# gillesdegottex/percivaltts

Measured on AMD Instinct MI355X. Metric: acoustic frames/sec per WGAN-GP critic+gen step, higher is better.
Workload: dtype f32

## Files before the change

### percivaltts_amd/csrc/dense.hip

```cpp
#include "common.h"
#include <cstdlib>

namespace ptts {
namespace dns {

typedef __bf16 bf16x8 __attribute__((ext_vector_type(8)));
typedef __bf16 bf16x4 __attribute__((ext_vector_type(4)));
typedef __bf16 bf16x2 __attribute__((ext_vector_type(2)));
typedef float f32x4 __attribute__((ext_vector_type(4)));
typedef float f32x2 __attribute__((ext_vector_type(2)));
typedef unsigned u32x2 __attribute__((ext_vector_type(2)));
typedef unsigned short u16;

constexpr int THREADS = 512;
constexpr int NBLK = 256;
constexpr int BK = 32;

#define DNS_PRODUCTS(X) X(2, 0) X(1, 1) X(0, 2) X(1, 0) X(0, 1) X(0, 0)
#define DNS_PRODUCTS_NPL(NPL, X) do { if (NPL == 3) { X(2, 0) X(1, 1) X(0, 2) X(1, 0) X(0, 1) } X(0, 0) } while (0)

__device__ __forceinline__ unsigned pk_bf16(float a, float b) {
    return __builtin_bit_cast(unsigned, __builtin_convertvector((f32x2){a, b}, bf16x2));
}
__device__ __forceinline__ void split3_pair(float a, float b, unsigned& p1, unsigned& p2, unsigned& p3) {
    p1 = pk_bf16(a, b);
    const float ra = a - __builtin_bit_cast(float, p1 << 16), rb = b - __builtin_bit_cast(float, p1 & 0xffff0000u);
    p2 = pk_bf16(ra, rb);
    const float sa = ra - __builtin_bit_cast(float, p2 << 16), sb = rb - __builtin_bit_cast(float, p2 & 0xffff0000u);
    p3 = pk_bf16(sa, sb);
}
__device__ __forceinline__ float max_fast(float a, float b) {
    float r;
    asm("v_max_f32 %0, %1, %2" : "=v"(r) : "v"(a), "v"(b));
    return r;
}

__global__ __launch_bounds__(256) void split3_dense_weight_kernel(const float* __restrict__ w, long long ldw, int K, int N,
                                                                  int transposed, u16* __restrict__ planes, int NT, int KS) {
    const long long idx = (long long)blockIdx.x * 256 + threadIdx.x;
    if (idx >= (long long)NT * KS * 64) return;
    const int lane = (int)(idx & 63);
    const long long t = idx >> 6;
    const int ks = (int)(t % KS), nt = (int)(t / KS);
    const int n = nt * 16 + (lane & 15), k0 = ks * 32 + (lane >> 4) * 8;
    float v[8];
#pragma unroll
    for (int e = 0; e < 8; ++e) {
        const int k = k0 + e;
        v[e] = (n < N && k < K) ? (transposed ? w[(long long)n * ldw + k] : w[(long long)k * ldw + n]) : 0.f;
    }
    unsigned q[3][4];
#pragma unroll
    for (int h = 0; h < 4; ++h) split3_pair(v[2 * h], v[2 * h + 1], q[0][h], q[1][h], q[2][h]);
    const size_t ps = (size_t)NT * KS * 512;
// ... 123 lines not shown
constexpr int SPL_ROW = 256 + 2;
__global__ __launch_bounds__(256) void split3_dense_weight_strided_lds_kernel(SplitStridedArgs a) {
    __shared__ float tile[32 * SPL_ROW];
    const int z = blockIdx.y, ks = blockIdx.x % a.KS, cb = blockIdx.x / a.KS;
    const float* __restrict__ w = a.w + (long long)z * a.stride_w;
    u16* __restrict__ planes = a.planes + (long long)z * a.stride_p;
    const int lane = threadIdx.x & 63, wave = threadIdx.x >> 6;
    const int n0 = cb * 256;
#pragma unroll
    for (int j = 0; j < 8; ++j) {
        const int r = wave + 4 * j, k = ks * 32 + r, n = n0 + 4 * lane;
        f32x4 v = {0.f, 0.f, 0.f, 0.f};
        if (k < a.K && n < a.N) v = *reinterpret_cast<const f32x4*>(w + (long long)k * a.ldw + n);
        float* d = tile + r * SPL_ROW + 4 * lane;
        d[0] = v[0]; d[1] = v[1]; d[2] = v[2]; d[3] = v[3];
    }
    __syncthreads();
    const size_t ps = (size_t)a.NT * a.KS * 512;
    const int li = lane & 15, lg = lane >> 4;
#pragma unroll
    for (int j = 0; j < 4; ++j) {
        const int ntl = wave + 4 * j;
        const int nt = cb * 16 + ntl;
        if (nt >= a.NT) continue;
        float v[8];
#pragma unroll
        for (int e = 0; e < 8; ++e) v[e] = tile[(8 * lg + e) * SPL_ROW + 16 * ntl + li];
        unsigned q[3][4];
#pragma unroll
        for (int h = 0; h < 4; ++h) split3_pair(v[2 * h], v[2 * h + 1], q[0][h], q[1][h], q[2][h]);
        const size_t idx = ((size_t)nt * a.KS + ks) * 64 + lane;
#pragma unroll
        for (int p = 0; p < 3; ++p)
            *reinterpret_cast<uint4*>(planes + p * ps + idx * 8) = make_uint4(q[p][0], q[p][1], q[p][2], q[p][3]);
    }
}

#ifndef DNS_DEPTH
#define DNS_DEPTH 2
#endif
struct DenseArgs {
    const float* A; const float* mask_src; const float* in_scale; const float* in_shift;
    const u16* planes; const float* bias; const float* out_mask; float* C;
    int M, N, K, NT, KS;
    long long lda, ldc;
    float alpha, out_alpha;
    int accumulate, has_affine, vec_out;
    const float* res; int res_rows; long long ldr;
    long long bsA, bsP, bsC;
    double* stats;
    const float* om_scale; const float* om_shift;
};

template <int MODE, bool AFFINE, int MT, int NPL>
__global__ __launch_bounds__(THREADS) void dense_bf16x6_kernel(DenseArgs g) {
    if (gridDim.z > 1) {
        g.A += (long long)blockIdx.z * g.bsA;
        g.planes += (long long)blockIdx.z * g.bsP;
        g.C += (long long)blockIdx.z * g.bsC;
    }
    constexpr int TBM = 16 * MT;
    constexpr int NA = (TBM * 8 + THREADS - 1) / THREADS;
    constexpr int ROWS = NA * THREADS / 8;
    constexpr int PL = ROWS * BK;
    constexpr bool MASK = MODE == PTTS_IN_MASKMUL;
    __shared__ __attribute__((aligned(16))) u16 As[2][NPL * PL];
    const int tid = threadIdx.x, lane = tid & 63;
    const int wave = __builtin_amdgcn_readfirstlane(tid >> 6);
    const int li = lane & 15, lg = lane >> 4;
    const int m0 = blockIdx.x * TBM, n0 = blockIdx.y * NBLK;
    const int KS = g.KS;
    const bool wave_live = n0 + 32 * wave < g.N;

    const int kq = tid & 7;
    const float* pa[NA]; const float* pm[NA]; bool oka[NA]; int dst[NA];
#pragma unroll
    for (int j = 0; j < NA; ++j) {
        const int row = (tid + j * THREADS) >> 3;
        oka[j] = row < TBM && m0 + row < g.M;
        const long long base = (long long)(oka[j] ? m0 + row : 0) * g.lda + 4 * kq;
        pa[j] = g.A + base;
        pm[j] = MASK ? g.mask_src + base : nullptr;
        dst[j] = row * BK + ((((kq >> 1) ^ ((row >> 1) & 2))) << 3) + (kq & 1) * 4;
    }
    struct Stage { f32x4 va[NA], vm[MASK ? NA : 1], sc, sh; bool kok; };
    auto load_a = [&](int s, Stage& sg) {
        const int k = s * BK + 4 * kq;
        sg.kok = k < g.K;
        const int ko = sg.kok ? s * BK : -4 * kq;
#pragma unroll
        for (int j = 0; j < NA; ++j) {
            sg.va[j] = *reinterpret_cast<const f32x4*>(pa[j] + ko);
            if (MASK) sg.vm[j] = *reinterpret_cast<const f32x4*>(pm[j] + ko);
        }
        if (AFFINE) {
            sg.sc = *reinterpret_cast<const f32x4*>(g.in_scale + (sg.kok ? k : 0));
            sg.sh = *reinterpret_cast<const f32x4*>(g.in_shift + (sg.kok ? k : 0));
        }
    };
    auto commit = [&](const Stage& sg, u16* as) {
        const f32x4 z4 = {0.f, 0.f, 0.f, 0.f};
#pragma unroll
        for (int j = 0; j < NA; ++j) {
            f32x4 a = sg.va[j];
            if (MODE == PTTS_IN_LRELU) {
                if (AFFINE) a = a * sg.sc + sg.sh;
// ... 34 lines not shown

    f32x4 acc[MT][2];
#pragma unroll
    for (int i = 0; i < MT; ++i) { acc[i][0] = f32x4{0.f, 0.f, 0.f, 0.f}; acc[i][1] = f32x4{0.f, 0.f, 0.f, 0.f}; }
    const int boff = li * BK + ((lg ^ ((li >> 1) & 2)) << 3);
    auto mfma_rows = [&](const u16* as, const bf16x8 (&wf)[2][NPL], int i0, int i1) {
#pragma unroll
        for (int i = i0; i < i1; ++i) {
            bf16x8 bf[NPL];
#pragma unroll
            for (int p = 0; p < NPL; ++p) bf[p] = *reinterpret_cast<const bf16x8*>(as + p * PL + boff + i * 16 * BK);
#define DNS_MM(PA, PW)                                                                                    \
            acc[i][0] = __builtin_amdgcn_mfma_f32_16x16x32_bf16(wf[0][PW < NPL ? PW : 0], bf[PA < NPL ? PA : 0], acc[i][0], 0, 0, 0);    \
            acc[i][1] = __builtin_amdgcn_mfma_f32_16x16x32_bf16(wf[1][PW < NPL ? PW : 0], bf[PA < NPL ? PA : 0], acc[i][1], 0, 0, 0);
            DNS_PRODUCTS_NPL(NPL, DNS_MM);
#undef DNS_MM
        }
    };

    constexpr int DEPTH = DNS_DEPTH;
    Stage sg[DEPTH];
    bf16x8 wc[2][NPL], wn[2][NPL];
#pragma unroll
    for (int j = 0; j < DEPTH; ++j) load_a(j, sg[j]);
    load_w(0, wc);
    commit(sg[0], As[0]);
    load_a(DEPTH, sg[0]);
    __syncthreads();
    auto step = [&](int s, int cut, Stage& nx) {
        const u16* as = As[s & 1];
        load_w(s + 1 < KS ? s + 1 : s, wn);
        mfma_rows(as, wc, 0, cut);
        commit(nx, As[(s + 1) & 1]);
        load_a(s + 1 + DEPTH, nx);
        mfma_rows(as, wc, cut, MT);
#pragma unroll
        for (int j = 0; j < 2; ++j)
#pragma unroll
            for (int p = 0; p < NPL; ++p) wc[j][p] = wn[j][p];
        __syncthreads();
    };
    auto run = [&](int cut) {
        int s = 0;
        for (; s + DEPTH <= KS; s += DEPTH) {
#pragma unroll
            for (int j = 0; j < DEPTH; ++j) step(s + j, cut, sg[(j + 1) % DEPTH]);
        }
#pragma unroll
        for (int j = 0; j < DEPTH; ++j)
            if (s + j < KS) step(s + j, cut, sg[(j + 1) % DEPTH]);
    };
    if (wave < 4) run(2); else run(MT - 2);
    if (!wave_live) return;
    const bool interior = m0 + TBM <= g.M;
    if (!g.vec_out) {
#pragma unroll
        for (int j = 0; j < 2; ++j)
#pragma unroll
            for (int i = 0; i < MT; ++i) {
                const int m = m0 + 16 * i + li;
                if (m >= g.M) continue;
#pragma unroll
                for (int e = 0; e < 4; ++e) {
                    const int n = n0 + 32 * wave + 16 * j + 4 * lg + e;
                    if (n >= g.N) continue;
                    const long long off = (long long)m * g.ldc + n;
                    float v = acc[i][j][e] + (g.bias ? g.bias[n] : 0.f);
                    if (g.out_mask) v *= g.out_mask[off] > 0.f ? 1.f : g.out_alpha;
                    if (g.res) { int mr = m; while (mr >= g.res_rows) mr -= g.res_rows; v += g.res[(long long)mr * g.ldr + n]; }
                    g.C[off] = v;
                }
            }
        return;
    }
#pragma unroll
    for (int j = 0; j < 2; ++j) {
        const int n = n0 + 32 * wave + 16 * j + 4 * lg;
        if (n >= g.N) continue;
        f32x4 bv = {0.f, 0.f, 0.f, 0.f};
        if (g.bias) bv = *reinterpret_cast<const f32x4*>(g.bias + n);
        const long long off0 = (long long)(m0 + li) * g.ldc + n;
        auto res_at = [&](int m) { int mr = m; while (mr >= g.res_rows) mr -= g.res_rows; return g.res + (long long)mr * g.ldr + n; };
        f32x4 ssum = {0.f, 0.f, 0.f, 0.f}, ssq = {0.f, 0.f, 0.f, 0.f};
        f32x4 osc = {1.f, 1.f, 1.f, 1.f}, osh = {0.f, 0.f, 0.f, 0.f};
        if (g.om_scale) { osc = *reinterpret_cast<const f32x4*>(g.om_scale + n); osh = *reinterpret_cast<const f32x4*>(g.om_shift + n); }
        auto aff_store = [&](f32x4& v, const f32x4& z) {
#pragma unroll
            for (int e = 0; e < 4; ++e) {
                const float gd = v[e] * ((z[e] * osc[e] + osh[e]) > 0.f ? 1.f : g.out_alpha);
                ssum[e] += gd * z[e]; ssq[e] += gd;
                v[e] = gd * osc[e];
            }
        };
        if (interior) {
            f32x4 mk[MT], old[MT];
            if (g.out_mask) {
#pragma unroll
                for (int i = 0; i < MT; ++i) mk[i] = *reinterpret_cast<const f32x4*>(g.out_mask + off0 + (long long)16 * i * g.ldc);
            }
            if (g.res) {
#pragma unroll
                for (int i = 0; i < MT; ++i) old[i] = *reinterpret_cast<const f32x4*>(res_at(m0 + 16 * i + li));
            }
#pragma unroll
            for (int i = 0; i < MT; ++i) {
                f32x4 v = acc[i][j] + bv;
                if (g.om_scale) {
                    aff_store(v, mk[i]);
                } else if (g.out_mask) {
#pragma unroll
                    for (int e = 0; e < 4; ++e) v[e] = v[e] * (mk[i][e] > 0.f ? 1.f : g.out_alpha);
                }
                if (g.res) v += old[i];
                if (g.stats && !g.om_scale) { ssum += v; ssq += v * v; }
                *reinterpret_cast<f32x4*>(g.C + off0 + (long long)16 * i * g.ldc) = v;
            }
        } else {
#pragma unroll
            for (int i = 0; i < MT; ++i) {
                const int m = m0 + 16 * i + li;
                if (m >= g.M) continue;
                const long long off = off0 + (long long)16 * i * g.ldc;
                f32x4 v = acc[i][j] + bv;
                if (g.out_mask) {
                    const f32x4 mk = *reinterpret_cast<const f32x4*>(g.out_mask + off);
                    if (g.om_scale) {
                        aff_store(v, mk);
                    } else {
#pragma unroll
                        for (int e = 0; e < 4; ++e) v[e] = v[e] * (mk[e] > 0.f ? 1.f : g.out_alpha);
                    }
                }
                if (g.res) v += *reinterpret_cast<const f32x4*>(res_at(m));
                if (g.stats && !g.om_scale) { ssum += v; ssq += v * v; }
                *reinterpret_cast<f32x4*>(g.C + off) = v;
            }
        }
        if (g.stats) {
#pragma unroll
            for (int e = 0; e < 4; ++e)
#pragma unroll
                for (int m = 1; m < 16; m <<= 1) { ssum[e] += __shfl_xor(ssum[e], m, 64); ssq[e] += __shfl_xor(ssq[e], m, 64); }
            if (li == 0) {
                double* row = g.stats + (size_t)blockIdx.x * 2 * g.N;
#pragma unroll
                for (int e = 0; e < 4; ++e) { row[n + e] = (double)ssum[e]; row[g.N + n + e] = (double)ssq[e]; }
            }
        }
    }
}

static int pick_mt(int M, int col_blocks) {
    static int forced = -1;
    if (forced < 0) { const char* e = getenv("PTTS_DENSE_MT"); forced = e ? atoi(e) : 0; }
    if (forced >= 4 && forced <= 8) return forced;
    int best = 8; double best_eff = -1.0;
    for (int mt = 4; mt <= 8; ++mt) {
        const long long blocks = (long long)((M + 16 * mt - 1) / (16 * mt)) * col_blocks;
        const long long rounds = (blocks + 255) / 256;
        const double eff = (double)M * col_blocks / (double)(rounds * 256 * 16 * mt);
        if (eff > best_eff + 1e-9) { best_eff = eff; best = mt; }
    }
    return best;
}


typedef short s16x4 __attribute__((ext_vector_type(4)));
typedef s16x4 __attribute__((address_space(3)))* lds_s16x4_ptr;
__device__ __forceinline__ bf16x4 tr_read(const u16* p) {
    return __builtin_bit_cast(bf16x4, __builtin_amdgcn_ds_read_tr16_b64_v4i16((lds_s16x4_ptr)(p)));
}
__device__ __forceinline__ bf16x8 cat8(bf16x4 a, bf16x4 b) { return __builtin_shufflevector(a, b, 0, 1, 2, 3, 4, 5, 6, 7); }

struct WgradArgs {
    const float* A; const float* dY; const float* mask_src; const float* in_scale; const float* in_shift;
    float* partials;
    int Kin, N, M;
    long long lda, ldb;
    float alpha;
    int tiles_n, steps_total, split;
};

constexpr int WT = 128;
constexpr int WROW = WT;
constexpr int WPL = 32 * WROW;
constexpr int WPART = WT * WT + WT;

template <int MODE, bool AFFINE, int NPL>
__global__ __launch_bounds__(THREADS) void dense_wgrad_bf16x6_kernel(WgradArgs g) {
    constexpr bool MASK = MODE == PTTS_IN_MASKMUL;
    extern __shared__ __attribute__((aligned(16))) u16 lds_w[];
    const int tid = threadIdx.x, lane = tid & 63;
    const int wave = __builtin_amdgcn_readfirstlane(tid >> 6);
    const int li = lane & 15, lg = lane >> 4;
    const int tile = blockIdx.y, tk = tile / g.tiles_n, tn = tile - tk * g.tiles_n;
    const int k0 = tk * WT, n0 = tn * WT;
    const int per = (g.steps_total + g.split - 1) / g.split;
    const int s_begin = blockIdx.x * per, s_end = min(g.steps_total, s_begin + per);
    const int nsteps = max(0, s_end - s_begin);

    const int c4 = tid & 31;
    const bool a_ok = k0 + 4 * c4 < g.Kin, d_ok = n0 + 4 * c4 < g.N;
    const float* pa = g.A + (a_ok ? k0 + 4 * c4 : 0);
    const float* pm = MASK ? g.mask_src + (a_ok ? k0 + 4 * c4 : 0) : nullptr;
    const float* pd = g.dY + (d_ok ? n0 + 4 * c4 : 0);
    int dst[2];
#pragma unroll
    for (int j = 0; j < 2; ++j) {
        const int row = (tid + j * THREADS) >> 5;
        dst[j] = row * WROW + ((((c4 >> 2) + row + 4 * (row >> 3)) & 7) << 4) + (c4 & 3) * 4;
    }
    f32x4 sc = {1.f, 1.f, 1.f, 1.f}, sh = {0.f, 0.f, 0.f, 0.f};
    if (AFFINE && a_ok) { sc = *reinterpret_cast<const f32x4*>(g.in_scale + k0 + 4 * c4); sh = *reinterpret_cast<const f32x4*>(g.in_shift + k0 + 4 * c4); }
    struct Stage { f32x4 va[2], vm[MASK ? 2 : 1], vd[2]; bool ok[2]; };
// ... 285 lines not shown
}

extern "C" int ptts_dense_bf16x6_stats(const float* A, const void* planes, const float* bias, float* C, int M, int N, int K,
                                       long long lda, long long ldc, int in_mode, const float* in_scale, const float* in_shift,
                                       float alpha, double* stats, int capacity_rows, int* nrows_out, void* stream) {
    PTTS_REQUIRE(stats && nrows_out && capacity_rows > 0, "dense_bf16x6_stats: no room for the sums");
    return dense_launch(A, planes, bias, C, M, N, K, lda, ldc, in_mode, in_scale, in_shift, nullptr, alpha, nullptr, 0, 0, nullptr,
                        stats, capacity_rows, nrows_out, stream);
}
extern "C" int ptts_dense_bf16x6_bwd_affine(const float* A, const void* planes, float* C, int M, int N, int K, long long lda, long long ldc,
                                            const float* z, const float* scale, const float* shift, float alpha,
                                            double* stats, int capacity_rows, int* nrows_out, void* stream) {
    PTTS_REQUIRE(z && scale && shift && stats && nrows_out && capacity_rows > 0, "dense_bf16x6_bwd_affine: null pointer");
    PTTS_REQUIRE((((uintptr_t)scale | (uintptr_t)shift) & 15) == 0, "dense_bf16x6_bwd_affine: scale / shift must be 16-byte aligned");
    g_om_scale = scale; g_om_shift = shift;
    const int rc = dense_launch(A, planes, nullptr, C, M, N, K, lda, ldc, PTTS_IN_NONE, nullptr, nullptr, nullptr, alpha, nullptr, 0, 0, z,
                                stats, capacity_rows, nrows_out, stream);
    g_om_scale = g_om_shift = nullptr;
    return rc;
}
extern "C" int ptts_dense_bf16x6_stats_rows(int M, int N) {
    if (M <= 0 || N <= 0) return 0;
    const int mt = pick_mt(M, (N + NBLK - 1) / NBLK);
    return (M + 16 * mt - 1) / (16 * mt);
}

static int dense_launch(const float* A, const void* planes, const float* bias, float* C, int M, int N, int K,
                        long long lda, long long ldc, int in_mode, const float* in_scale, const float* in_shift,
                        const float* mask_src, float alpha, const float* res, int res_rows, long long ldr,
                        const float* out_mask, double* stats, int stats_capacity_rows, int* stats_rows_out, void* stream) {
    const int accumulate = res != nullptr;
    PTTS_REQUIRE(!res || (res_rows > 0 && ldr >= N && M <= 8LL * res_rows), "dense_bf16x6: bad residual (rows %d, ldr %lld)", res_rows, ldr);
    PTTS_REQUIRE(A && planes && C, "dense_bf16x6: null matrix");
    PTTS_REQUIRE(ptts_dense_bf16x6_supported(M, N, K, lda, ldc), "dense_bf16x6: unsupported shape M=%d N=%d K=%d lda=%lld ldc=%lld (K and lda must be multiples of 4)", M, N, K, lda, ldc);
    PTTS_REQUIRE(lda >= K && ldc >= N, "dense_bf16x6: bad leading dims");
    PTTS_REQUIRE(in_mode >= 0 && in_mode <= 2, "dense_bf16x6: bad in_mode %d", in_mode);
    PTTS_REQUIRE((in_scale == nullptr) == (in_shift == nullptr), "dense_bf16x6: scale/shift must come together");
    PTTS_REQUIRE(in_mode != PTTS_IN_MASKMUL || mask_src, "dense_bf16x6: MASKMUL needs mask_src");
    PTTS_REQUIRE(in_mode == PTTS_IN_LRELU || !in_scale, "dense_bf16x6: scale/shift need PTTS_IN_LRELU");
    PTTS_REQUIRE(!(out_mask && bias), "dense_bf16x6: out_mask with bias is not defined");
    PTTS_REQUIRE(alpha >= 0.f && alpha <= 1.f, "dense_bf16x6: LeakyReLU slope %g outside [0, 1]", alpha);
    const bool vec_out = N % 4 == 0 && ldc % 4 == 0 && ((uintptr_t)C & 15) == 0 && (!bias || ((uintptr_t)bias & 15) == 0) &&
                         (!out_mask || ((uintptr_t)out_mask & 15) == 0) && (!res || (((uintptr_t)res & 15) == 0 && ldr % 4 == 0));
    PTTS_REQUIRE(((uintptr_t)A & 15) == 0 && (!mask_src || ((uintptr_t)mask_src & 15) == 0) &&
                 (!in_scale || (((uintptr_t)in_scale | (uintptr_t)in_shift) & 15) == 0), "dense_bf16x6: A, its mask and scale/shift must be 16-byte aligned");
    DenseArgs g;
    g.A = A; g.mask_src = mask_src; g.in_scale = in_scale; g.in_shift = in_shift; g.planes = (const u16*)planes; g.bias = bias;
    g.out_mask = out_mask; g.C = C; g.M = M; g.N = N; g.K = K;
    g.NT = (N + NBLK - 1) / NBLK * (NBLK / 16); g.KS = (K + BK - 1) / BK;
    g.lda = lda; g.ldc = ldc; g.alpha = alpha; g.out_alpha = alpha; g.accumulate = accumulate; g.has_affine = in_scale != nullptr; g.vec_out = vec_out;
    g.res = res; g.res_rows = res ? res_rows : 1; g.ldr = ldr;
    g.bsA = g.bsP = g.bsC = 0;
    const int cb = (N + NBLK - 1) / NBLK;
    const int mt = pick_mt(M, cb);
    const dim3 grid((unsigned)((M + 16 * mt - 1) / (16 * mt)), (unsigned)cb);
    g.stats = stats;
    g.om_scale = g_om_scale; g.om_shift = g_om_shift;
    if (stats) {
        PTTS_REQUIRE(vec_out, "dense_bf16x6_stats: N and ldc must be multiples of 4, C (and bias) 16-byte aligned");
        PTTS_REQUIRE(stats_capacity_rows >= (int)grid.x, "dense_bf16x6_stats: room for %d rows of sums, %d needed", stats_capacity_rows, (int)grid.x);
        *stats_rows_out = (int)grid.x;
    }
    hipStream_t st = (hipStream_t)stream;
    const bool one = ptts::bf16_products();
#define DNS_L(MODE, AFF, MT) do { if (one) hipLaunchKernelGGL((dense_bf16x6_kernel<MODE, AFF, MT, 1>), grid, dim3(THREADS), 0, st, g); \
                                  else hipLaunchKernelGGL((dense_bf16x6_kernel<MODE, AFF, MT, 3>), grid, dim3(THREADS), 0, st, g); } while (0)
#define DNS_M(MT)                                                                \
    do {                                                                         \
        if (in_mode == PTTS_IN_LRELU) { if (in_scale) DNS_L(PTTS_IN_LRELU, true, MT); else DNS_L(PTTS_IN_LRELU, false, MT); } \
        else if (in_mode == PTTS_IN_MASKMUL) DNS_L(PTTS_IN_MASKMUL, false, MT);  \
        else DNS_L(PTTS_IN_NONE, false, MT);                                     \
    } while (0)
    switch (mt) {
        case 4: DNS_M(4); break;
        case 5: DNS_M(5); break;
        case 6: DNS_M(6); break;
        case 7: DNS_M(7); break;
        default: DNS_M(8); break;
    }
#undef DNS_M
#undef DNS_L
    return check_launch("dense_bf16x6");
}

extern "C" int ptts_conv1d_freq_kernel_planes(const float* w, const float* tw, void* planes, int NB, int KW, int Cin, int N, int Kh,
                                              void* stream) {
    PTTS_REQUIRE(w && tw && planes && NB > 0 && Cin > 0 && N > 0, "conv1d_freq_kernel_planes: bad arguments");
    PTTS_REQUIRE(Kh >= Cin && Kh % 8 == 0, "conv1d_freq_kernel_planes: Kh=%d must be a multiple of 8 and >= Cin=%d", Kh, Cin);
    const int NT = (N + NBLK - 1) / NBLK * (NBLK / 16), KS = (2 * Kh + BK - 1) / BK;
    const long long total = (long long)NT * KS * 64;
    const long long fstride = (long long)(ptts_dense_planes_bytes(N, 2 * Kh) / sizeof(u16));
    const dim3 grid((unsigned)((total + 255) / 256), (unsigned)((NB + WDFT_FCH - 1) / WDFT_FCH));
#define WDFT(KWv) hipLaunchKernelGGL(conv1d_wdft_planes_kernel<KWv>, grid, dim3(256), 0, (hipStream_t)stream, w, tw, (u16*)planes, fstride, NB, Cin, N, Kh, NT, KS)
    switch (KW) {
        case 3: WDFT(3); break;
        case 5: WDFT(5); break;
        case 7: WDFT(7); break;
        case 9: WDFT(9); break;
        case 11: WDFT(11); break;
        case 21: WDFT(21); break;
        default: set_error("conv1d_freq_kernel_planes: KW=%d not instantiated (3, 5, 7, 9, 11, 21)", KW); return PTTS_EINVAL;
    }
#undef WDFT
    return check_launch("conv1d_freq_kernel_planes");
}

extern "C" int ptts_dense_bf16x6_batched(const float* A, long long strideA, const void* planes, long long stride_planes_bytes,
                                         const float* bias, float* C, long long strideC, int nbatch, int M, int N, int K,
                                         long long lda, long long ldc, int planes_count, void* stream) {
    PTTS_REQUIRE(A && planes && C && nbatch > 0 && nbatch <= 65535, "dense_bf16x6_batched: bad arguments");
    PTTS_REQUIRE(ptts_dense_bf16x6_supported(M, N, K, lda, ldc), "dense_bf16x6_batched: unsupported shape M=%d N=%d K=%d lda=%lld ldc=%lld", M, N, K, lda, ldc);
    PTTS_REQUIRE(lda >= K && ldc >= N && planes_count >= 1 && planes_count <= 3 && planes_count != 2, "dense_bf16x6_batched: bad leading dims / planes");
    PTTS_REQUIRE(stride_planes_bytes % 16 == 0 && strideA % 4 == 0 && ((uintptr_t)A & 15) == 0, "dense_bf16x6_batched: strides of A / planes must keep 16-byte alignment");
    const bool vec_out = N % 4 == 0 && ldc % 4 == 0 && strideC % 4 == 0 && ((uintptr_t)C & 15) == 0 && (!bias || ((uintptr_t)bias & 15) == 0);
    DenseArgs g;
    g.A = A; g.mask_src = nullptr; g.in_scale = nullptr; g.in_shift = nullptr; g.planes = (const u16*)planes; g.bias = bias;
    g.out_mask = nullptr; g.C = C; g.M = M; g.N = N; g.K = K;
    g.NT = (N + NBLK - 1) / NBLK * (NBLK / 16); g.KS = (K + BK - 1) / BK;
    g.lda = lda; g.ldc = ldc; g.alpha = 0.f; g.out_alpha = 0.f; g.accumulate = 0; g.has_affine = 0; g.vec_out = vec_out;
    g.res = nullptr; g.res_rows = 1; g.ldr = 0;
    g.bsA = strideA; g.bsP = stride_planes_bytes / 2; g.bsC = strideC;
    g.stats = nullptr; g.om_scale = g.om_shift = nullptr;
    const int cb = (N + NBLK - 1) / NBLK;
    int mt = 8; double best_eff = -1.0;
    {
        static int forced = -1;
        if (forced < 0) { const char* e = getenv("PTTS_DENSE_BATCHED_MT"); forced = e ? atoi(e) : 0; }
        for (int m = 8; m >= 4; --m) {
            const int tiles = (M + 16 * m - 1) / (16 * m);
            const double eff = (double)M / (double)(tiles * 16 * m);
            if (eff > best_eff + 1e-9) { best_eff = eff; mt = m; }
        }
        if (forced >= 4 && forced <= 8) mt = forced;
    }
    const dim3 grid((unsigned)((M + 16 * mt - 1) / (16 * mt)), (unsigned)cb, (unsigned)nbatch);
    hipStream_t st = (hipStream_t)stream;
    const bool one = planes_count == 1;
#define DNS_B(MT) do { if (one) hipLaunchKernelGGL((dense_bf16x6_kernel<PTTS_IN_NONE, false, MT, 1>), grid, dim3(THREADS), 0, st, g); \
                       else hipLaunchKernelGGL((dense_bf16x6_kernel<PTTS_IN_NONE, false, MT, 3>), grid, dim3(THREADS), 0, st, g); } while (0)
    switch (mt) {
        case 4: DNS_B(4); break;
        case 5: DNS_B(5); break;
        case 6: DNS_B(6); break;
        case 7: DNS_B(7); break;
        default: DNS_B(8); break;
    }
#undef DNS_B
    return check_launch("dense_bf16x6_batched");
}

extern "C" int ptts_dense_wgrad_bf16x6_supported(int Kin, int N, int M, long long lda, long long ldb) {
    return (Kin > 0 && N > 0 && M > 0 && Kin % 4 == 0 && N % 4 == 0 && lda % 4 == 0 && ldb % 4 == 0 &&
            (long long)((Kin + WT - 1) / WT) * ((N + WT - 1) / WT) <= 65535) ? 1 : 0;
}

namespace {
int wgrad_split(int Kin, int N, int M) {
    const int tiles = ((Kin + WT - 1) / WT) * ((N + WT - 1) / WT), steps = (M + 31) / 32;
    int split = (256 + tiles - 1) / tiles;
    static int env_split = -1;
    if (env_split < 0) { const char* e = getenv("PTTS_DENSE_WGRAD_SPLIT"); env_split = e ? atoi(e) : 0; }
    if (env_split > 0) split = env_split;
    if (split > steps) split = steps;
    return split < 1 ? 1 : split;
}
}

extern "C" size_t ptts_dense_wgrad_workspace_bytes(int Kin, int N, int M) {
    if (Kin <= 0 || N <= 0 || M <= 0) return 0;
    const size_t tiles = (size_t)((Kin + WT - 1) / WT) * ((N + WT - 1) / WT);
    return tiles * wgrad_split(Kin, N, M) * WPART * sizeof(float);
}

extern "C" int ptts_dense_wgrad_bf16x6_partials(const float* A, const float* dY, const float* mask_src, const float* in_scale,
                                                const float* in_shift, void* workspace, size_t workspace_bytes, int* split_out,
                                                int Kin, int N, int M, long long lda, long long ldb, int in_mode, float alpha,
                                                void* stream) {
    PTTS_REQUIRE(A && dY && workspace && split_out, "dense_wgrad_bf16x6: null pointer");
    PTTS_REQUIRE(ptts_dense_wgrad_bf16x6_supported(Kin, N, M, lda, ldb), "dense_wgrad_bf16x6: unsupported shape Kin=%d N=%d M=%d lda=%lld ldb=%lld", Kin, N, M, lda, ldb);
    PTTS_REQUIRE(lda >= Kin && ldb >= N, "dense_wgrad_bf16x6: bad leading dims");
    PTTS_REQUIRE(in_mode >= 0 && in_mode <= 2, "dense_wgrad_bf16x6: bad in_mode %d", in_mode);
    PTTS_REQUIRE((in_scale == nullptr) == (in_shift == nullptr), "dense_wgrad_bf16x6: scale/shift must come together");
    PTTS_REQUIRE(in_mode != PTTS_IN_MASKMUL || mask_src, "dense_wgrad_bf16x6: MASKMUL needs mask_src");
    PTTS_REQUIRE(in_mode == PTTS_IN_LRELU || !in_scale, "dense_wgrad_bf16x6: scale/shift need PTTS_IN_LRELU");
    PTTS_REQUIRE(alpha >= 0.f && alpha <= 1.f, "dense_wgrad_bf16x6: LeakyReLU slope %g outside [0, 1]", alpha);
    PTTS_REQUIRE(((uintptr_t)A & 15) == 0 && ((uintptr_t)dY & 15) == 0 && (!mask_src || ((uintptr_t)mask_src & 15) == 0) &&
                 (!in_scale || (((uintptr_t)in_scale | (uintptr_t)in_shift) & 15) == 0), "dense_wgrad_bf16x6: operands must be 16-byte aligned");
    const size_t need = ptts_dense_wgrad_workspace_bytes(Kin, N, M);
    if (workspace_bytes < need) { set_error("dense_wgrad_bf16x6: workspace %zu < %zu", workspace_bytes, need); return PTTS_EWORKSPACE; }
    WgradArgs g;
    g.A = A; g.dY = dY; g.mask_src = mask_src; g.in_scale = in_scale; g.in_shift = in_shift; g.partials = (float*)workspace;
    g.Kin = Kin; g.N = N; g.M = M; g.lda = lda; g.ldb = ldb; g.alpha = alpha;
    const int tiles_k = (Kin + WT - 1) / WT;
    g.tiles_n = (N + WT - 1) / WT;
    g.steps_total = (M + 31) / 32;
    const int tiles = tiles_k * g.tiles_n;
    g.split = wgrad_split(Kin, N, M);
    *split_out = g.split;
    const dim3 grid((unsigned)g.split, (unsigned)tiles);
    hipStream_t st = (hipStream_t)stream;
// ... 53 lines not shown
```

Baseline: 4.648 million.

## Add persistent streaming dense kernel that walks multiple M tiles per workgroup

Adds a persistent-style variant of the bf16x6 dense GEMM kernel. Each workgroup loops over several M tiles with a continuous software pipeline across tile boundaries, and the grid width is chosen from the CU count to cut wave-quantization rounds. The tile size is picked by a new cost model that also counts a fixed per-tile overhead. The store epilogue is factored into a shared helper that can process rows in chunks, which limits register pressure. The risks are longer per-block runtimes, extra register use and fewer concurrent blocks when the cost model misjudges.

```diff
diff --git a/percivaltts_amd/csrc/dense.hip b/percivaltts_amd/csrc/dense.hip
--- a/percivaltts_amd/csrc/dense.hip
+++ b/percivaltts_amd/csrc/dense.hip
@@ -1,5 +1,6 @@
 #include "common.h"
 #include <cstdlib>
+#include <type_traits>
 
 namespace ptts {
 namespace dns {
@@ -229,6 +230,115 @@
     const float* om_scale; const float* om_shift;
 };
 
+template <int MT, int CH = MT>
+__device__ __forceinline__ void dense_store_tile(const DenseArgs& g, const f32x4 (&acc)[MT][2], int m0, int n0, int wave, int li, int lg,
+                                                 int tile) {
+    constexpr int TBM = 16 * MT;
+    const bool interior = m0 + TBM <= g.M;
+    if (!g.vec_out) {
+#pragma unroll
+        for (int j = 0; j < 2; ++j)
+#pragma unroll
+            for (int i = 0; i < MT; ++i) {
+                const int m = m0 + 16 * i + li;
+                if (m >= g.M) continue;
+#pragma unroll
+                for (int e = 0; e < 4; ++e) {
+                    const int n = n0 + 32 * wave + 16 * j + 4 * lg + e;
+                    if (n >= g.N) continue;
+                    const long long off = (long long)m * g.ldc + n;
+                    float v = acc[i][j][e] + (g.bias ? g.bias[n] : 0.f);
+                    if (g.out_mask) v *= g.out_mask[off] > 0.f ? 1.f : g.out_alpha;
+                    if (g.res) { int mr = m; while (mr >= g.res_rows) mr -= g.res_rows; v += g.res[(long long)mr * g.ldr + n]; }
+                    g.C[off] = v;
+                }
+            }
+        return;
+    }
+#pragma unroll
+    for (int j = 0; j < 2; ++j) {
+        const int n = n0 + 32 * wave + 16 * j + 4 * lg;
+        if (n >= g.N) continue;
+        f32x4 bv = {0.f, 0.f, 0.f, 0.f};
+        if (g.bias) bv = *reinterpret_cast<const f32x4*>(g.bias + n);
+        const long long off0 = (long long)(m0 + li) * g.ldc + n;
+        auto res_at = [&](int m) { int mr = m; while (mr >= g.res_rows) mr -= g.res_rows; return g.res + (long long)mr * g.ldr + n; };
+        f32x4 ssum = {0.f, 0.f, 0.f, 0.f}, ssq = {0.f, 0.f, 0.f, 0.f};
+        f32x4 osc = {1.f, 1.f, 1.f, 1.f}, osh = {0.f, 0.f, 0.f, 0.f};
+        if (g.om_scale) { osc = *reinterpret_cast<const f32x4*>(g.om_scale + n); osh = *reinterpret_cast<const f32x4*>(g.om_shift + n); }
+        auto aff_store = [&](f32x4& v, const f32x4& z) {
+#pragma unroll
+            for (int e = 0; e < 4; ++e) {
+                const float gd = v[e] * ((z[e] * osc[e] + osh[e]) > 0.f ? 1.f : g.out_alpha);
+                ssum[e] += gd * z[e]; ssq[e] += gd;
+                v[e] = gd * osc[e];
+            }
+        };
+        if (interior) {
+#pragma unroll
+            for (int i0 = 0; i0 < MT; i0 += CH) {
+                f32x4 mk[CH], old[CH];
+                if (g.out_mask) {
+#pragma unroll
+                    for (int c = 0; c < CH; ++c)
+                        if (i0 + c < MT) mk[c] = *reinterpret_cast<const f32x4*>(g.out_mask + off0 + (long long)16 * (i0 + c) * g.ldc);
+                }
+                if (g.res) {
+#pragma unroll
+                    for (int c = 0; c < CH; ++c)
+                        if (i0 + c < MT) old[c] = *reinterpret_cast<const f32x4*>(res_at(m0 + 16 * (i0 + c) + li));
+                }
+#pragma unroll
+                for (int c = 0; c < CH; ++c) {
+                    const int i = i0 + c;
+                    if (i >= MT) break;
+                    f32x4 v = acc[i][j] + bv;
+                    if (g.om_scale) {
+                        aff_store(v, mk[c]);
+                    } else if (g.out_mask) {
+#pragma unroll
+                        for (int e = 0; e < 4; ++e) v[e] = v[e] * (mk[c][e] > 0.f ? 1.f : g.out_alpha);
+                    }
+                    if (g.res) v += old[c];
+                    if (g.stats && !g.om_scale) { ssum += v; ssq += v * v; }
+                    *reinterpret_cast<f32x4*>(g.C + off0 + (long long)16 * i * g.ldc) = v;
+                }
+            }
+        } else {
+#pragma unroll
+            for (int i = 0; i < MT; ++i) {
+                const int m = m0 + 16 * i + li;
+                if (m >= g.M) continue;
+                const long long off = off0 + (long long)16 * i * g.ldc;
+                f32x4 v = acc[i][j] + bv;
+                if (g.out_mask) {
+                    const f32x4 mk = *reinterpret_cast<const f32x4*>(g.out_mask + off);
+                    if (g.om_scale) {
+                        aff_store(v, mk);
+                    } else {
+#pragma unroll
+                        for (int e = 0; e < 4; ++e) v[e] = v[e] * (mk[e] > 0.f ? 1.f : g.out_alpha);
+                    }
+                }
+                if (g.res) v += *reinterpret_cast<const f32x4*>(res_at(m));
+                if (g.stats && !g.om_scale) { ssum += v; ssq += v * v; }
+                *reinterpret_cast<f32x4*>(g.C + off) = v;
+            }
+        }
+        if (g.stats) {
+#pragma unroll
+            for (int e = 0; e < 4; ++e)
+#pragma unroll
+                for (int m = 1; m < 16; m <<= 1) { ssum[e] += __shfl_xor(ssum[e], m, 64); ssq[e] += __shfl_xor(ssq[e], m, 64); }
+            if (li == 0) {
+                double* row = g.stats + (size_t)tile * 2 * g.N;
+#pragma unroll
+                for (int e = 0; e < 4; ++e) { row[n + e] = (double)ssum[e]; row[g.N + n + e] = (double)ssq[e]; }
+            }
+        }
+    }
+}
+
 template <int MODE, bool AFFINE, int MT, int NPL>
 __global__ __launch_bounds__(THREADS) void dense_bf16x6_kernel(DenseArgs g) {
     if (gridDim.z > 1) {
@@ -369,114 +479,226 @@
     };
     if (wave < 4) run(2); else run(MT - 2);
     if (!wave_live) return;
-    const bool interior = m0 + TBM <= g.M;
-    if (!g.vec_out) {
+    dense_store_tile<MT>(g, acc, m0, n0, wave, li, lg, blockIdx.x);
+}
+
+template <int MODE, bool AFFINE, int MT, int NPL>
+__global__ __launch_bounds__(THREADS) void dense_bf16x6_stream_kernel(DenseArgs g) {
+    if (gridDim.z > 1) {
+        g.A += (long long)blockIdx.z * g.bsA;
+        g.planes += (long long)blockIdx.z * g.bsP;
+        g.C += (long long)blockIdx.z * g.bsC;
+    }
+    constexpr int TBM = 16 * MT;
+    constexpr int NA = (TBM * 8 + THREADS - 1) / THREADS;
+    constexpr int ROWS = NA * THREADS / 8;
+    constexpr int PL = ROWS * BK;
+    constexpr bool MASK = MODE == PTTS_IN_MASKMUL;
+    __shared__ __attribute__((aligned(16))) u16 As[2][NPL * PL];
+    const int tid = threadIdx.x, lane = tid & 63;
+    const int wave = __builtin_amdgcn_readfirstlane(tid >> 6);
+    const int li = lane & 15, lg = lane >> 4;
+    const int n0 = blockIdx.y * NBLK;
+    const int KS = g.KS;
+    const int gx = gridDim.x, tiles = (g.M + TBM - 1) / TBM;
+    const int ntiles = (tiles - (int)blockIdx.x + gx - 1) / gx;
+    const bool wave_live = n0 + 32 * wave < g.N;
+    auto tile_m0 = [&](int i) { return ((int)blockIdx.x + i * gx) * TBM; };
+    auto advance = [&](int& i, int& s, int d) { s += d; while (s >= KS) { s -= KS; ++i; } };
+
+    const int kq = tid & 7;
+    auto slot_row = [&](int j) { return (tid + j * THREADS) >> 3; };
+    auto row_ok = [&](int m0, int j) { return slot_row(j) < TBM && m0 + slot_row(j) < g.M; };
+    struct Stage { f32x4 va[NA], vm[MASK ? NA : 1], sc, sh; };
+    auto load_a = [&](int i, int s, Stage& sg) __attribute__((always_inline)) {
+        const int m0 = tile_m0(i);
+        const int k = s * BK + 4 * kq;
+        const bool kok = k < g.K;
+#pragma unroll
+        for (int j = 0; j < NA; ++j) {
+            const bool rok = row_ok(m0, j);
+            const long long off = (long long)(rok ? m0 + slot_row(j) : 0) * g.lda + (kok ? k : 0);
+            sg.va[j] = *reinterpret_cast<const f32x4*>(g.A + off);
+            if (MASK) sg.vm[j] = *reinterpret_cast<const f32x4*>(g.mask_src + off);
+        }
+        if (AFFINE) {
+            sg.sc = *reinterpret_cast<const f32x4*>(g.in_scale + (kok ? k : 0));
+            sg.sh = *reinterpret_cast<const f32x4*>(g.in_shift + (kok ? k : 0));
+        }
+    };
+    auto commit = [&](int i, int s, const Stage& sg, u16* as) __attribute__((always_inline)) {
+        const f32x4 z4 = {0.f, 0.f, 0.f, 0.f};
+        const int m0 = tile_m0(i);
+        const bool kok = s * BK + 4 * kq < g.K;
+#pragma unroll
+        for (int j = 0; j < NA; ++j) {
+            const bool ok = row_ok(m0, j) && kok;
+            const int row = slot_row(j);
+            f32x4 a = sg.va[j];
+            if (MODE == PTTS_IN_LRELU) {
+                if (AFFINE) a = a * sg.sc + sg.sh;
+                if (!ok) a = z4;
+#pragma unroll
+                for (int e = 0; e < 4; ++e) a[e] = max_fast(a[e], g.alpha * a[e]);
+            } else if (MASK) {
+                if (!ok) a = z4;
+#pragma unroll
+                for (int e = 0; e < 4; ++e) a[e] = a[e] * (sg.vm[j][e] > 0.f ? 1.f : g.alpha);
+            } else {
+                if (!ok) a = z4;
+            }
+            u16* d = as + row * BK + ((((kq >> 1) ^ ((row >> 1) & 2))) << 3) + (kq & 1) * 4;
+            if (NPL == 3) {
+                unsigned a1, a2, a3, b1, b2, b3;
+                split3_pair(a[0], a[1], a1, a2, a3);
+                split3_pair(a[2], a[3], b1, b2, b3);
+                *reinterpret_cast<u32x2*>(d) = (u32x2){a1, b1};
+                *reinterpret_cast<u32x2*>(d + PL) = (u32x2){a2, b2};
+                *reinterpret_cast<u32x2*>(d + 2 * PL) = (u32x2){a3, b3};
+            } else {
+                *reinterpret_cast<u32x2*>(d) = (u32x2){pk_bf16(a[0], a[1]), pk_bf16(a[2], a[3])};
+            }
+        }
+    };
+
+    const size_t ps = (size_t)g.NT * KS * 512;
+    const u16* wp[2];
+#pragma unroll
+    for (int j = 0; j < 2; ++j) wp[j] = g.planes + (((size_t)((n0 >> 4) + 2 * (wave_live ? wave : 0) + j) * KS) * 64 + lane) * 8;
+    auto load_w = [&](int s, bf16x8 (&wf)[2][NPL]) {
 #pragma unroll
         for (int j = 0; j < 2; ++j)
 #pragma unroll
-            for (int i = 0; i < MT; ++i) {
-                const int m = m0 + 16 * i + li;
-                if (m >= g.M) continue;
-#pragma unroll
-                for (int e = 0; e < 4; ++e) {
-                    const int n = n0 + 32 * wave + 16 * j + 4 * lg + e;
-                    if (n >= g.N) continue;
-                    const long long off = (long long)m * g.ldc + n;
-                    float v = acc[i][j][e] + (g.bias ? g.bias[n] : 0.f);
-                    if (g.out_mask) v *= g.out_mask[off] > 0.f ? 1.f : g.out_alpha;
-                    if (g.res) { int mr = m; while (mr >= g.res_rows) mr -= g.res_rows; v += g.res[(long long)mr * g.ldr + n]; }
-                    g.C[off] = v;
-                }
-            }
-        return;
-    }
-#pragma unroll
-    for (int j = 0; j < 2; ++j) {
-        const int n = n0 + 32 * wave + 16 * j + 4 * lg;
-        if (n >= g.N) continue;
-        f32x4 bv = {0.f, 0.f, 0.f, 0.f};
-        if (g.bias) bv = *reinterpret_cast<const f32x4*>(g.bias + n);
-        const long long off0 = (long long)(m0 + li) * g.ldc + n;
-        auto res_at = [&](int m) { int mr = m; while (mr >= g.res_rows) mr -= g.res_rows; return g.res + (long long)mr * g.ldr + n; };
-        f32x4 ssum = {0.f, 0.f, 0.f, 0.f}, ssq = {0.f, 0.f, 0.f, 0.f};
-        f32x4 osc = {1.f, 1.f, 1.f, 1.f}, osh = {0.f, 0.f, 0.f, 0.f};
-        if (g.om_scale) { osc = *reinterpret_cast<const f32x4*>(g.om_scale + n); osh = *reinterpret_cast<const f32x4*>(g.om_shift + n); }
-        auto aff_store = [&](f32x4& v, const f32x4& z) {
-#pragma unroll
-            for (int e = 0; e < 4; ++e) {
-                const float gd = v[e] * ((z[e] * osc[e] + osh[e]) > 0.f ? 1.f : g.out_alpha);
-                ssum[e] += gd * z[e]; ssq[e] += gd;
-                v[e] = gd * osc[e];
-            }
-        };
-        if (interior) {
-            f32x4 mk[MT], old[MT];
-            if (g.out_mask) {
-#pragma unroll
-                for (int i = 0; i < MT; ++i) mk[i] = *reinterpret_cast<const f32x4*>(g.out_mask + off0 + (long long)16 * i * g.ldc);
-            }
-            if (g.res) {
-#pragma unroll
-                for (int i = 0; i < MT; ++i) old[i] = *reinterpret_cast<const f32x4*>(res_at(m0 + 16 * i + li));
-            }
-#pragma unroll
-            for (int i = 0; i < MT; ++i) {
-                f32x4 v = acc[i][j] + bv;
-                if (g.om_scale) {
-                    aff_store(v, mk[i]);
-                } else if (g.out_mask) {
-#pragma unroll
-                    for (int e = 0; e < 4; ++e) v[e] = v[e] * (mk[i][e] > 0.f ? 1.f : g.out_alpha);
-                }
-                if (g.res) v += old[i];
-                if (g.stats && !g.om_scale) { ssum += v; ssq += v * v; }
-                *reinterpret_cast<f32x4*>(g.C + off0 + (long long)16 * i * g.ldc) = v;
-            }
-        } else {
-#pragma unroll
-            for (int i = 0; i < MT; ++i) {
-                const int m = m0 + 16 * i + li;
-                if (m >= g.M) continue;
-                const long long off = off0 + (long long)16 * i * g.ldc;
-                f32x4 v = acc[i][j] + bv;
-                if (g.out_mask) {
-                    const f32x4 mk = *reinterpret_cast<const f32x4*>(g.out_mask + off);
-                    if (g.om_scale) {
-                        aff_store(v, mk);
-                    } else {
-#pragma unroll
-                        for (int e = 0; e < 4; ++e) v[e] = v[e] * (mk[e] > 0.f ? 1.f : g.out_alpha);
-                    }
-                }
-                if (g.res) v += *reinterpret_cast<const f32x4*>(res_at(m));
-                if (g.stats && !g.om_scale) { ssum += v; ssq += v * v; }
-                *reinterpret_cast<f32x4*>(g.C + off) = v;
-            }
-        }
-        if (g.stats) {
-#pragma unroll
-            for (int e = 0; e < 4; ++e)
-#pragma unroll
-                for (int m = 1; m < 16; m <<= 1) { ssum[e] += __shfl_xor(ssum[e], m, 64); ssq[e] += __shfl_xor(ssq[e], m, 64); }
-            if (li == 0) {
-                double* row = g.stats + (size_t)blockIdx.x * 2 * g.N;
-#pragma unroll
-                for (int e = 0; e < 4; ++e) { row[n + e] = (double)ssum[e]; row[g.N + n + e] = (double)ssq[e]; }
-            }
-        }
-    }
-}
-
-static int pick_mt(int M, int col_blocks) {
+            for (int p = 0; p < NPL; ++p) wf[j][p] = *reinterpret_cast<const bf16x8*>(wp[j] + p * ps + (size_t)s * 512);
+    };
+
+    f32x4 acc[MT][2];
+#pragma unroll
+    for (int i = 0; i < MT; ++i) { acc[i][0] = f32x4{0.f, 0.f, 0.f, 0.f}; acc[i][1] = f32x4{0.f, 0.f, 0.f, 0.f}; }
+    const int boff = li * BK + ((lg ^ ((li >> 1) & 2)) << 3);
+    auto mfma_rows = [&](const u16* as, const bf16x8 (&wf)[2][NPL], int i0, int i1) __attribute__((always_inline)) {
+#pragma unroll
+        for (int i = i0; i < i1; ++i) {
+            bf16x8 bf[NPL];
+#pragma unroll
+            for (int p = 0; p < NPL; ++p) bf[p] = *reinterpret_cast<const bf16x8*>(as + p * PL + boff + i * 16 * BK);
+#define DNS_MM(PA, PW)                                                                                    \
+            acc[i][0] = __builtin_amdgcn_mfma_f32_16x16x32_bf16(wf[0][PW < NPL ? PW : 0], bf[PA < NPL ? PA : 0], acc[i][0], 0, 0, 0);    \
+            acc[i][1] = __builtin_amdgcn_mfma_f32_16x16x32_bf16(wf[1][PW < NPL ? PW : 0], bf[PA < NPL ? PA : 0], acc[i][1], 0, 0, 0);
+            DNS_PRODUCTS_NPL(NPL, DNS_MM);
+#undef DNS_MM
+        }
+    };
+
+    constexpr int DEPTH = DNS_DEPTH;
+    static_assert(DEPTH == 1 || DEPTH == 2, "dense_bf16x6_stream_kernel: DNS_DEPTH 1 or 2");
+    Stage sg[DEPTH];
+    bf16x8 wc[2][NPL], wn[2][NPL];
+    {
+        int i = 0, s = 0;
+#pragma unroll
+        for (int j = 0; j < DEPTH; ++j) { load_a(i, s, sg[j]); advance(i, s, 1); }
+        load_w(0, wc);
+        commit(0, 0, sg[0], As[0]);
+        load_a(i, s, sg[0]);
+    }
+    __syncthreads();
+    auto step = [&](int i, int s, int cut, Stage& nx) __attribute__((always_inline)) {
+        const int u = i * KS + s;
+        const u16* as = As[u & 1];
+        load_w(s + 1 < KS ? s + 1 : 0, wn);
+        mfma_rows(as, wc, 0, cut);
+        int i1 = i, s1 = s;
+        advance(i1, s1, 1);
+        commit(i1, s1, nx, As[(u + 1) & 1]);
+        int i2 = i, s2 = s;
+        advance(i2, s2, 1 + DEPTH);
+        load_a(i2, s2, nx);
+        mfma_rows(as, wc, cut, MT);
+#pragma unroll
+        for (int j = 0; j < 2; ++j)
+#pragma unroll
+            for (int p = 0; p < NPL; ++p) wc[j][p] = wn[j][p];
+        __syncthreads();
+    };
+    auto run_tile = [&](auto ph, int i, int cut) __attribute__((always_inline)) {
+        constexpr int PH = decltype(ph)::value;
+        int s = 0;
+        for (; s + DEPTH <= KS; s += DEPTH) {
+#pragma unroll
+            for (int j = 0; j < DEPTH; ++j) step(i, s + j, cut, sg[(PH + j + 1) % DEPTH]);
+        }
+#pragma unroll
+        for (int j = 0; j < DEPTH; ++j)
+            if (s + j < KS) step(i, s + j, cut, sg[(PH + j + 1) % DEPTH]);
+    };
+    typedef std::integral_constant<int, 0> ph0;
+    typedef std::integral_constant<int, 1 % DEPTH> ph1;
+    for (int i = 0; i < ntiles; ++i) {
+        const bool odd = ((i * KS) % DEPTH) != 0;
+        if (wave < 4) { if (odd) run_tile(ph1(), i, 2); else run_tile(ph0(), i, 2); }
+        else { if (odd) run_tile(ph1(), i, MT - 2); else run_tile(ph0(), i, MT - 2); }
+        if (wave_live) dense_store_tile<MT, 2>(g, acc, tile_m0(i), n0, wave, li, lg, (int)blockIdx.x + i * gx);
+#pragma unroll
+        for (int r = 0; r < MT; ++r) { acc[r][0] = f32x4{0.f, 0.f, 0.f, 0.f}; acc[r][1] = f32x4{0.f, 0.f, 0.f, 0.f}; }
+    }
+}
+
+static int forced_mt() {
     static int forced = -1;
     if (forced < 0) { const char* e = getenv("PTTS_DENSE_MT"); forced = e ? atoi(e) : 0; }
-    if (forced >= 4 && forced <= 8) return forced;
+    return forced >= 4 && forced <= 8 ? forced : 0;
+}
+static int pick_mt(int M, int col_blocks) {
+    if (forced_mt()) return forced_mt();
     int best = 8; double best_eff = -1.0;
     for (int mt = 4; mt <= 8; ++mt) {
         const long long blocks = (long long)((M + 16 * mt - 1) / (16 * mt)) * col_blocks;
         const long long rounds = (blocks + 255) / 256;
         const double eff = (double)M * col_blocks / (double)(rounds * 256 * 16 * mt);
         if (eff > best_eff + 1e-9) { best_eff = eff; best = mt; }
+    }
+    return best;
+}
+
+static bool dense_stream_on() {
+    const char* e = getenv("PTTS_DENSE_STREAM");
+    return !e || atoi(e) != 0;
+}
+static int resident_workgroups() {
+    static int r = 0;
+    if (r <= 0) {
+        int dev = 0, cus = 0;
+        if (hipGetDevice(&dev) != hipSuccess || hipDeviceGetAttribute(&cus, hipDeviceAttributeMultiprocessorCount, dev) != hipSuccess || cus <= 0) cus = 256;
+        r = cus;
+    }
+    return r;
+}
+static int stream_gx(int T, long long others, long long* cost) {
+    const long long R = resident_workgroups();
+    long long best = -1;
+    int best_gx = T;
+    for (int t = 1; t <= T && (best < 0 || t <= best); ++t) {
+        const int gx = (T + t - 1) / t;
+        const long long walk = (T + gx - 1) / gx, rounds = ((long long)gx * others + R - 1) / R;
+        const long long c = rounds * walk;
+        if (best < 0 || c < best || (c == best && gx < best_gx)) { best = c; best_gx = gx; }
+    }
+    if (cost) *cost = best;
+    return best_gx;
+}
+#ifndef DNS_TILE_ROWS_FIXED
+#define DNS_TILE_ROWS_FIXED 8
+#endif
+static int pick_mt_stream(int M, long long others, int mt_max) {
+    if (forced_mt()) return forced_mt();
+    int best = mt_max;
+    long long best_rows = -1;
+    for (int mt = mt_max; mt >= 4; --mt) {
+        long long c = 0;
+        stream_gx((M + 16 * mt - 1) / (16 * mt), others, &c);
+        const long long rows = c * (16 * mt + DNS_TILE_ROWS_FIXED);
+        if (best_rows < 0 || rows < best_rows) { best_rows = rows; best = mt; }
     }
     return best;
 }
@@ -868,19 +1090,24 @@
     g.res = res; g.res_rows = res ? res_rows : 1; g.ldr = ldr;
     g.bsA = g.bsP = g.bsC = 0;
     const int cb = (N + NBLK - 1) / NBLK;
-    const int mt = pick_mt(M, cb);
-    const dim3 grid((unsigned)((M + 16 * mt - 1) / (16 * mt)), (unsigned)cb);
+    bool stream_form = dense_stream_on();
+    const int mt = (stream_form && !stats) ? pick_mt_stream(M, cb, in_scale || in_mode == PTTS_IN_MASKMUL ? 6 : 8) : pick_mt(M, cb);
+    const int tiles = (M + 16 * mt - 1) / (16 * mt);
+    const int gx = stream_form ? stream_gx(tiles, cb, nullptr) : tiles;
+    stream_form = stream_form && gx < tiles;
+    const dim3 grid((unsigned)gx, (unsigned)cb);
     g.stats = stats;
     g.om_scale = g_om_scale; g.om_shift = g_om_shift;
     if (stats) {
         PTTS_REQUIRE(vec_out, "dense_bf16x6_stats: N and ldc must be multiples of 4, C (and bias) 16-byte aligned");
-        PTTS_REQUIRE(stats_capacity_rows >= (int)grid.x, "dense_bf16x6_stats: room for %d rows of sums, %d needed", stats_capacity_rows, (int)grid.x);
-        *stats_rows_out = (int)grid.x;
+        PTTS_REQUIRE(stats_capacity_rows >= tiles, "dense_bf16x6_stats: room for %d rows of sums, %d needed", stats_capacity_rows, tiles);
+        *stats_rows_out = tiles;
     }
     hipStream_t st = (hipStream_t)stream;
     const bool one = ptts::bf16_products();
-#define DNS_L(MODE, AFF, MT) do { if (one) hipLaunchKernelGGL((dense_bf16x6_kernel<MODE, AFF, MT, 1>), grid, dim3(THREADS), 0, st, g); \
-                                  else hipLaunchKernelGGL((dense_bf16x6_kernel<MODE, AFF, MT, 3>), grid, dim3(THREADS), 0, st, g); } while (0)
+#define DNS_K(MODE, AFF, MT, NPL) do { if (stream_form) hipLaunchKernelGGL((dense_bf16x6_stream_kernel<MODE, AFF, MT, NPL>), grid, dim3(THREADS), 0, st, g); \
+                                       else hipLaunchKernelGGL((dense_bf16x6_kernel<MODE, AFF, MT, NPL>), grid, dim3(THREADS), 0, st, g); } while (0)
+#define DNS_L(MODE, AFF, MT) do { if (one) DNS_K(MODE, AFF, MT, 1); else DNS_K(MODE, AFF, MT, 3); } while (0)
 #define DNS_M(MT)                                                                \
     do {                                                                         \
         if (in_mode == PTTS_IN_LRELU) { if (in_scale) DNS_L(PTTS_IN_LRELU, true, MT); else DNS_L(PTTS_IN_LRELU, false, MT); } \
@@ -896,6 +1123,7 @@
     }
 #undef DNS_M
 #undef DNS_L
+#undef DNS_K
     return check_launch("dense_bf16x6");
 }
 
@@ -949,11 +1177,15 @@
         }
         if (forced >= 4 && forced <= 8) mt = forced;
     }
-    const dim3 grid((unsigned)((M + 16 * mt - 1) / (16 * mt)), (unsigned)cb, (unsigned)nbatch);
+    const int tiles = (M + 16 * mt - 1) / (16 * mt);
+    const int gx = dense_stream_on() ? stream_gx(tiles, (long long)cb * nbatch, nullptr) : tiles;
+    const bool stream_form = gx < tiles;
+    const dim3 grid((unsigned)gx, (unsigned)cb, (unsigned)nbatch);
     hipStream_t st = (hipStream_t)stream;
     const bool one = planes_count == 1;
-#define DNS_B(MT) do { if (one) hipLaunchKernelGGL((dense_bf16x6_kernel<PTTS_IN_NONE, false, MT, 1>), grid, dim3(THREADS), 0, st, g); \
-                       else hipLaunchKernelGGL((dense_bf16x6_kernel<PTTS_IN_NONE, false, MT, 3>), grid, dim3(THREADS), 0, st, g); } while (0)
+#define DNS_K(MT, NPL) do { if (stream_form) hipLaunchKernelGGL((dense_bf16x6_stream_kernel<PTTS_IN_NONE, false, MT, NPL>), grid, dim3(THREADS), 0, st, g); \
+                            else hipLaunchKernelGGL((dense_bf16x6_kernel<PTTS_IN_NONE, false, MT, NPL>), grid, dim3(THREADS), 0, st, g); } while (0)
+#define DNS_B(MT) do { if (one) DNS_K(MT, 1); else DNS_K(MT, 3); } while (0)
     switch (mt) {
         case 4: DNS_B(4); break;
         case 5: DNS_B(5); break;
@@ -962,6 +1194,7 @@
         default: DNS_B(8); break;
     }
 #undef DNS_B
+#undef DNS_K
     return check_launch("dense_bf16x6_batched");
 }
 
```

Result: no change. 4.656 million (median of 6 runs) (+0.2%).
